# sashakolpakov/graphem-rapids

Hardware: AMD Instinct MI355X
Metric: layout iterations/s (higher is better)
Workload: dtype f32; 1 GPU; rr1m; graph=rr, n_vertices=1000000, n_edges=4000000, n_components=3, n_neighbors=10, sample_size=256, sampler=device, knn=auto, knn_distance=exact, parallelism=rows/1, reference_identical=False

## Files before the change

graphem-rapids_amd/csrc/common.h:

```cpp
#pragma once
#include <hip/hip_runtime.h>
#include <stdint.h>

#include "dispatch.h"

#define GH_WAVE 64
#ifndef GH_DEPTH8
#define GH_DEPTH8 4
#endif
#ifndef GH_DEPTH16
#define GH_DEPTH16 2
#endif
#define GH_GATHER_DEPTH(LD) ((LD) <= 4 ? 8 : (LD) <= 8 ? GH_DEPTH8 : GH_DEPTH16)

template <int D>
__device__ __forceinline__ float gh_sumsq(const float *x) {
    float s = 0.0f;
    int d = 0;
    if constexpr (D >= 8) {
        float acc[8];
#pragma unroll
        for (int l = 0; l < 8; ++l) acc[l] = 0.0f;
#pragma unroll
        for (d = 0; d + 8 <= D; d += 8) {
// ... 32 lines not shown
__device__ __forceinline__ void gh_load_row(const float *__restrict__ pos, int64_t v, float *out) {
    const float4 *p = reinterpret_cast<const float4 *>(pos + v * LD);
#pragma unroll
    for (int i = 0; i < LD / 4; ++i) {
        const float4 t = p[i];
        out[4 * i + 0] = t.x; out[4 * i + 1] = t.y; out[4 * i + 2] = t.z; out[4 * i + 3] = t.w;
    }
}

template <int LD>
__device__ __forceinline__ void gh_store_row(float *__restrict__ dst, int64_t v, const float *in) {
    float4 *p = reinterpret_cast<float4 *>(dst + v * LD);
#pragma unroll
    for (int i = 0; i < LD / 4; ++i) p[i] = make_float4(in[4 * i], in[4 * i + 1], in[4 * i + 2], in[4 * i + 3]);
}

__device__ __forceinline__ uint64_t gh_key(float d2, uint32_t id) {
    return (static_cast<uint64_t>(__float_as_uint(d2)) << 32) | id;
}
__device__ __forceinline__ float gh_key_d2(uint64_t k) { return __uint_as_float(static_cast<uint32_t>(k >> 32)); }
__device__ __forceinline__ uint32_t gh_key_id(uint64_t k) { return static_cast<uint32_t>(k); }

#define GH_KEY_INF 0xFFFFFFFFFFFFFFFFull

__device__ __forceinline__ double gh_wave_sum(double v) {
#pragma unroll
    for (int off = 32; off > 0; off >>= 1) v += __shfl_down(v, off, GH_WAVE);
    return v;
}

__device__ __forceinline__ float gh_sqrt_ieee(float x) {
    if (__builtin_expect(!(x >= 0x1p-96f), 0)) return sqrtf(x);
    const float s = __builtin_amdgcn_sqrtf(x);
    const float sm = __uint_as_float(__float_as_uint(s) - 1u), sp = __uint_as_float(__float_as_uint(s) + 1u);
    const float rm = fmaf(-sm, s, x), rp = fmaf(-sp, s, x);
    float out = rm <= 0.0f ? sm : s;
    out = rp > 0.0f ? sp : out;
    return x == INFINITY ? x : out;
}
template <int D>
__device__ __forceinline__ void gh_div_by(const float (&n)[D], float d, float (&q)[D]) {
    uint32_t emin = 255;
#pragma unroll
    for (int i = 0; i < D; ++i) emin = min(emin, (__float_as_uint(n[i]) >> 23) & 0xFFu);
    if (__builtin_expect(!(d >= 0x1p-40f && d <= 0x1p20f) || emin < 27u, 0)) {
#pragma unroll
// ... 144 lines not shown
```

graphem-rapids_amd/csrc/engine.h:

```cpp
#pragma once
#include <hip/hip_runtime.h>
#include <stdint.h>
#include <memory>
#include <string>
#include <vector>

#include "../../include/graphem_hip.h"
#include "host_util.h"
#include "step_plan.h"
#include "exchange_layout.h"

#define GH_CAND_CAP 16384
#define GH_SEL_BUF 4096
#define GH_SEL_CHUNK 2048
#define GH_CNT_STRIDE 32
#define GH_POS_PAD_ROWS 1024
#define GH_CT_M 64
#define GH_CT_EMPTY 0xFFFFFFFFu

struct gh_timer_slot {
    std::string name;
    double total_ms = 0.0;
    int64_t launches = 0;
    std::vector<std::pair<hipEvent_t, hipEvent_t>> pending;
// ... 145 lines not shown

    int grid_G = 0, grid_bits = 0;
    int64_t grid_cells = 0;
    size_t grid_temp_bytes = 0;
    gh_dev<uint32_t> d_grid_u32;
    gh_dev<float> d_grid_smid;
    gh_dev<unsigned char> d_grid_temp;

    gh_dev<double> d_blockstats;
    int nblocks_update = 0;
    gh_dev<double> d_stats_buf;
    double *d_stats = nullptr;

    gh_dev<unsigned> d_tau_flag;
    gh_dev<uint32_t> d_qcell;
    gh_dev<unsigned> d_qc_flag;
    unsigned qc_epoch = 0;
    gh_dev<int32_t> d_wait_failed;
    gh_dev<uint32_t> d_cmin;
    bool cmin_dirty[2] = {false, false};


#define GH_STAMP_EXTRA 8192
    gh_dev<unsigned long long> d_stamps;
    bool timing = false;
    std::vector<gh_timer_slot> timers;

    std::unique_ptr<gh_ivf, gh_part_delete> ivf;
    std::unique_ptr<gh_f64, gh_part_delete> f64;
    std::unique_ptr<gh_comm, gh_part_delete> comm;
};

template <class T> gh_status gh_alloc(gh_engine *h, gh_dev<T> &buf, size_t count, bool zero) {
    if (count == 0) count = 1;
    if (!buf.alloc(count * sizeof(T))) {
        h->err = std::string("hipMalloc failed: ") + hipGetErrorString(hipGetLastError());
        return GH_ERR_NOMEM;
    }
    if (zero) GH_HIP(hipMemsetAsync(buf.p, 0, count * sizeof(T), h->stream));
    return GH_OK;
}

inline gh_ids gh_own_ids(const gh_engine *h) { return gh_ids{h->S >= h->E ? GH_IDS_ARANGE : GH_IDS_SAMPLER, h->d_sampled.p}; }
inline void gh_set_lookahead(gh_engine *h, const gh_ids *next) {
    h->lookahead.valid = next != nullptr;
    h->lookahead.rows = false;
// ... 5 lines not shown
    h->lookahead.src = next;
    h->lookahead.iter = h->iter + 1;
}
inline bool gh_lookahead_rows_for(const gh_engine *h, const gh_ids *next) {
    return next && h->lookahead.rows && h->lookahead.iter == h->iter + 1 && h->lookahead.src.mode == next->mode &&
           h->lookahead.src.ids == next->ids;
}
inline void gh_drop_lookahead_rows(gh_engine *h) { h->lookahead.rows = false; }
inline bool gh_lookahead_done_for(const gh_engine *h, const gh_ids &src) {
    return h->lookahead.valid && h->lookahead.iter == h->iter && h->lookahead.src.mode == src.mode && h->lookahead.src.ids == src.ids;
}
inline void gh_drop_lookahead(gh_engine *h) { h->lookahead.valid = false; }

inline void gh_step_reset(gh_engine *h) {
    h->step.new0_ready = h->step.stats_reduced = h->step.intersect_done = h->step.rows_early = false;
}
inline void gh_step_new0_ready(gh_engine *h) { h->step.new0_ready = true; }
inline void gh_step_stats_reduced(gh_engine *h) { h->step.stats_reduced = true; }
inline void gh_step_sums_spent(gh_engine *h) { h->step.new0_ready = h->step.stats_reduced = false; }
inline void gh_step_intersect_done(gh_engine *h) { h->step.intersect_done = true; }
inline void gh_step_tcount_reset_pending(gh_engine *h, bool pending) { h->step.tcount_reset_pending = pending; }
inline void gh_step_set_rows_early(gh_engine *h, bool early) { h->step.rows_early = early; }
inline void gh_step_own_ids(gh_engine *h, bool own) { h->step.own_ids = own; }

enum gh_finish_kind { GH_FINISH_OWN, GH_FINISH_OWN_ALL_STATS, GH_FINISH_ALL_ROWS };

struct gh_scope {
    gh_engine *h;
    int slot = -1;
    hipEvent_t a = nullptr, b = nullptr;
    hipStream_t stream = nullptr;
    gh_scope(gh_engine *h_, const char *name, hipStream_t on = nullptr );
    ~gh_scope();
};

struct gh_graph_plan {
    const int32_t *edges = nullptr;
    std::vector<int32_t> internal;
    std::vector<int32_t> rowptr, adj;
    std::vector<int32_t> first_edge, own_eids, vblock;
    std::vector<int32_t> long_rows, long_ownptr, long_ownadj, long_eptr, long_erow;
    std::vector<uint8_t> own_long;
    std::vector<int32_t> sub_uv;
};
void gh_plan_graph(gh_engine *h, const int32_t *edges, bool partitioned, int reorder, gh_graph_plan *g);
void gh_auto_knn_method(gh_engine *h);
// ... 64 lines not shown
```

graphem-rapids_amd/csrc/forces.hip:

```cpp
#include "common.h"
#include "engine.h"
#include "intersect_core.h"
#include "setup_core.h"

namespace {

template <int D, int LD, bool WRITE_MID, bool LONG>
__global__ __launch_bounds__(256) void spring_kernel(
    const float *__restrict__ pos, const int32_t *__restrict__ rowptr, const int32_t *__restrict__ adj,
    const int32_t *__restrict__ first_edge, int64_t edge_lo, int64_t row_lo, int64_t rows, float L_min,
    float neg_k, float *__restrict__ outF, int64_t f_row0, float *__restrict__ mid, gh_long_args la) {
    const int64_t i = blockIdx.x * (int64_t)blockDim.x + threadIdx.x;
    if (i >= rows) return;
    const int64_t x = row_lo + i;
    float px[LD], F[LD];
    gh_load_row<LD>(pos, x, px);
    int64_t mid_row0 = 0;
    if (WRITE_MID) mid_row0 = first_edge[i] - edge_lo;
    if constexpr (LONG)
        spring_row<D, LD, WRITE_MID>(pos, adj, rowptr[i], rowptr[i + 1], x, px, L_min, neg_k, F, mid, mid_row0, la, (int)i,
                                     outF + (i + f_row0) * LD);
    else
        spring_pull<D, LD, WRITE_MID>(pos, adj, rowptr[i], rowptr[i + 1], x, px, L_min, neg_k, F, mid, mid_row0);
    gh_store_row<LD>(outF, i + f_row0, F);
// ... 196 lines not shown
__global__ __launch_bounds__(256) void stats_reduce_kernel(const double *__restrict__ blockstats, int nblocks, int LD,
                                                          double *__restrict__ stats) {
    const int c = blockIdx.x;
    double s = 0.0;
    for (int b = threadIdx.x; b < nblocks; b += blockDim.x) s += blockstats[(int64_t)c * nblocks + b];
    __shared__ double red[4];
    const double a = gh_wave_sum(s);
    if ((threadIdx.x & 63) == 0) red[threadIdx.x >> 6] = a;
    __syncthreads();
    if (threadIdx.x == 0) stats[c] = ((red[0] + red[1]) + red[2]) + red[3];
}

template <int LD>
__global__ __launch_bounds__(256) void stats_fix_kernel(const double *__restrict__ blockstats, int nblocks,
                                                       const float *__restrict__ pos, const float *__restrict__ Fs,
                                                       const double *__restrict__ acc,
                                                       const int32_t *__restrict__ touched,
                                                       const int32_t *__restrict__ tcount, int64_t row_lo,
                                                       int64_t rows, float *__restrict__ out_new,
                                                       double *__restrict__ stats, int skip_reduce,
                                                       int32_t *__restrict__ patch_count = nullptr ,
                                                       float *__restrict__ patch_rows = nullptr, int patch_cap = 0,
                                                       gh_setup_args sa = gh_setup_args{} ,
                                                       const int32_t *__restrict__ tflag = nullptr, float *__restrict__ setup_rows = nullptr) {
    constexpr int NFIX = 2 * LD;
    if ((int)blockIdx.x >= NFIX) {
        gh_setup_gather<LD>(sa, gh_gather_src{pos, Fs, out_new, acc, tflag, setup_rows}, (int)blockIdx.x - NFIX);
        return;
    }
    __shared__ double red[4][2 * LD];
    const int lane = threadIdx.x & 63, w = threadIdx.x >> 6;
    if (!skip_reduce) {
        const int c = blockIdx.x;
        double s = 0.0;
        double s4[4] = {0.0, 0.0, 0.0, 0.0};
        const double *col = blockstats + (int64_t)c * nblocks;
        int b = threadIdx.x;
        for (; b + 3 * (int)blockDim.x < nblocks; b += 4 * blockDim.x) {
#pragma unroll
            for (int u = 0; u < 4; ++u) s4[u] += col[b + u * blockDim.x];
        }
        for (int u = 0; b < nblocks; b += blockDim.x, ++u) s4[u] += col[b];
        s = (s4[0] + s4[1]) + (s4[2] + s4[3]);
        const double a = gh_wave_sum(s);
        if (lane == 0) red[w][0] = a;
        __syncthreads();
        if (threadIdx.x == 0) stats[c] = ((red[0][0] + red[1][0]) + red[2][0]) + red[3][0];
        __syncthreads();
    }
    double dx[LD], dxx[LD];
#pragma unroll
    for (int d = 0; d < LD; ++d) { dx[d] = 0.0; dxx[d] = 0.0; }
    const int nt = *tcount;
    for (int t = blockIdx.x * blockDim.x + threadIdx.x; t < nt; t += NFIX * blockDim.x) {
        const int64_t x = touched[t];
        const int64_t i = x - row_lo;
        if (i < 0 || i >= rows) continue;
        float p[LD], f[LD], nw[LD];
        gh_load_row<LD>(pos, x, p);
        gh_load_row<LD>(Fs, i, f);
#pragma unroll
        for (int d = 0; d < LD; ++d) {
            const float n0 = p[d] + f[d];
            const float tot = f[d] + (float)acc[x * LD + d];
            nw[d] = p[d] + tot;
            dx[d] += (double)nw[d] - (double)n0;
            dxx[d] += (double)nw[d] * (double)nw[d] - (double)n0 * (double)n0;
        }
        if (!patch_count) gh_store_row<LD>(out_new, i, nw);
        else gh_patch_append<LD>(patch_count, patch_rows, patch_cap, x, nw);
    }
#pragma unroll
    for (int d = 0; d < LD; ++d) {
        const double a = gh_wave_sum(dx[d]), b = gh_wave_sum(dxx[d]);
        if (lane == 0) { red[w][d] = a; red[w][LD + d] = b; }
    }
    __syncthreads();
    if (threadIdx.x < 2 * LD)
        stats[(2 + 2 * blockIdx.x) * LD + threadIdx.x] =
            ((red[0][threadIdx.x] + red[1][threadIdx.x]) + red[2][threadIdx.x]) + red[3][threadIdx.x];
}

__device__ __forceinline__ void gh_clear_touched(double *__restrict__ acc, int32_t *__restrict__ tflag,
                                                 const int32_t *__restrict__ touched, const int32_t *__restrict__ tcount, int LD,
                                                 int64_t t0, int64_t T) {
    const int64_t nt = (int64_t)(*tcount) * LD;
    for (int64_t t = t0; t < nt; t += T) {
        const int64_t x = touched[t / LD];
        const int d = (int)(t % LD);
        acc[x * LD + d] = 0.0;
        if (d == 0) tflag[x] = 0;
    }
}

struct gh_norm_src {
    const float *rows;
    int64_t chunk;
    int64_t block;
    int RS;
    int64_t out_lo, out_rows;
    const double *stats;
    int world;
    int64_t stats_block;
// ... 393 lines not shown
    }
    if (!fused) return launch_mid_gather(h);
    return GH_OK;
}

gh_status gh_launch_mid_only(gh_engine *h) { return launch_mid_gather(h); }

gh_status gh_launch_integrate(gh_engine *h, const gh_ids *next) {
    gh_drop_lookahead_rows(h);
    const bool fused_sums = h->step.new0_ready && h->rows > 0, reduced = h->step.stats_reduced;
    gh_step_sums_spent(h);
    if (fused_sums) {
        gh_scope t(h, "stats_fix");
        gh_setup_args sa{};
        unsigned gather = 0;
        if (next && h->plan.stage_rows) {
            sa = gh_make_setup_args(h, *next, h->iter + 1);
            if (sa.tiles > 0) gather = gh_gather_blocks(sa.S);
        }
        if (!gh_dispatch_stride(h->LD, [&](auto ld) {
                stats_fix_kernel<ld()><<<dim3(gh_fix_blocks(ld()) + gather), dim3(256), 0, h->stream>>>(
                    h->d_blockstats.p, h->n_vblocks, h->d_pos.p, h->d_Fs.p, h->d_acc.p, h->d_touched.p, h->d_tcount.p, h->part.row_lo,
                    h->rows, h->d_new, h->d_stats, reduced ? 1 : 0,
                    gh_patch_count(h), gh_patch_records(h), (int)h->xch.lay.patch_cap, sa, h->d_tflag.p, h->d_setup_rows.p);
            })) {
            h->err = "stats_fix: the fused step left its sums for a row stride other than 4, 8 or 16";
            return GH_ERR_RUNTIME;
        }
        GH_LAUNCH_CHECK();
        if (gather) gh_set_lookahead_rows(h, *next);
        return GH_OK;
    }
    GH_HIP(hipMemsetAsync(h->d_stats + 2 * h->LD, 0, sizeof(double) * 2 * gh_fix_blocks(h->LD) * h->LD, h->stream));
    if (h->rows == 0) {
        GH_HIP(hipMemsetAsync(h->d_stats, 0, sizeof(double) * 2 * h->LD, h->stream));
        return GH_OK;
    }
    const unsigned grid = grid_for(h->rows, 256);
    int32_t *pc = gh_patch_count(h);
    float *pr = gh_patch_records(h);
    const int pcap = (int)h->xch.lay.patch_cap;
    float *wide_out = h->d_new;
    {
        gh_scope t(h, "integrate");
        if (!gh_dispatch_stride(h->LD, [&](auto ld) {
                integrate_kernel<ld()><<<dim3(grid), dim3(256), 0, h->stream>>>(h->d_pos.p, h->d_Fs.p, h->part.row_lo, h->rows, h->d_acc.p,
                                                                               h->d_tflag.p, h->d_new, h->d_blockstats.p, pc, pr, pcap);
// ... 238 lines not shown
```

graphem-rapids_amd/csrc/intersect_core.h:

```cpp
#pragma once
#include "common.h"

__host__ __device__ __forceinline__ float gh_orient2d(const float *a, const float *b, const float *c) {
    return (b[0] - a[0]) * (c[1] - a[1]) - (b[1] - a[1]) * (c[0] - a[0]);
}

__device__ inline void gh_intersect_pair(const float *__restrict__ pos, int D, int LD,
                                         const int32_t *__restrict__ edges, int32_t i, int32_t j, float k_inter,
                                         double *__restrict__ acc, int32_t *__restrict__ tflag,
                                         int32_t *__restrict__ touched, int32_t *__restrict__ tcount,
                                         float *__restrict__ diff, int32_t own_lo = 0, int32_t own_hi = 0x7FFFFFFF ) {
    if (!(i < j)) return;
    const int32_t v[4] = {edges[2 * (int64_t)i], edges[2 * (int64_t)i + 1], edges[2 * (int64_t)j], edges[2 * (int64_t)j + 1]};
    if (v[0] == v[2] || v[0] == v[3] || v[1] == v[2] || v[1] == v[3]) return;
    if (D < 2) return;
    const float *p1 = pos + (int64_t)v[0] * LD, *p2 = pos + (int64_t)v[1] * LD;
    const float *q1 = pos + (int64_t)v[2] * LD, *q2 = pos + (int64_t)v[3] * LD;
    const float o1 = gh_orient2d(p1, p2, q1), o2 = gh_orient2d(p1, p2, q2);
    const float o3 = gh_orient2d(q1, q2, p1), o4 = gh_orient2d(q1, q2, p2);
    if (!(o1 * o2 < 0.0f && o3 * o4 < 0.0f)) return;
    for (int role = 0; role < 4; ++role) {
        if (v[role] < own_lo || v[role] >= own_hi) continue;
        const float *x = pos + (int64_t)v[role] * LD;
        for (int d = 0; d < D; ++d) {
// ... 33 lines not shown
        for (int d = 0; d < D; ++d) diff[d] = x[role][d] - cen[d];
        const float dist = sqrtf(gh_sumsq<D>(diff)) + 1e-6f;
        const float dd = dist * dist;
#pragma unroll
        for (int d = 0; d < D; ++d) atomicAdd(&acc[(int64_t)v[role] * LD + d], (double)((k_inter * diff[d]) / dd));
        if (atomicExch(&tflag[v[role]], 1) == 0) touched[atomicAdd(tcount, 1)] = v[role];
    }
}

struct gh_pair_list {
    int n;
    int nt, base;
    int4 v[128];
    int32_t t[512];
};

template <int D, int LD>
__device__ __forceinline__ void gh_intersect_query_wide(const float *__restrict__ pos, const int32_t *__restrict__ edges,
                                                        int32_t i, const uint64_t *best , int k,
                                                        float k_inter, double *__restrict__ acc,
                                                        int32_t *__restrict__ tflag, int32_t *__restrict__ touched,
                                                        int32_t *__restrict__ tcount, gh_pair_list *pl,
                                                        int32_t *__restrict__ own_count = nullptr ,
                                                        int32_t own_lo = 0, int32_t own_hi = 0x7FFFFFFF) {
    if (threadIdx.x == 0) { pl->n = 0; pl->nt = 0; }
    __syncthreads();
    for (int c = threadIdx.x; c < k; c += blockDim.x) {
        const int32_t j = (int32_t)(uint32_t)best[c + 1];
        if (!(i < j)) continue;
        const int2 ei = reinterpret_cast<const int2 *>(edges)[i], ej = reinterpret_cast<const int2 *>(edges)[j];
        if (ei.x == ej.x || ei.x == ej.y || ei.y == ej.x || ei.y == ej.y) continue;
        const float2 a = *reinterpret_cast<const float2 *>(pos + (int64_t)ei.x * LD), b = *reinterpret_cast<const float2 *>(pos + (int64_t)ei.y * LD);
        const float2 p = *reinterpret_cast<const float2 *>(pos + (int64_t)ej.x * LD), q = *reinterpret_cast<const float2 *>(pos + (int64_t)ej.y * LD);
        const float x0[2] = {a.x, a.y}, x1[2] = {b.x, b.y}, x2[2] = {p.x, p.y}, x3[2] = {q.x, q.y};
        const float o1 = gh_orient2d(x0, x1, x2), o2 = gh_orient2d(x0, x1, x3);
        const float o3 = gh_orient2d(x2, x3, x0), o4 = gh_orient2d(x2, x3, x1);
        if (!(o1 * o2 < 0.0f && o3 * o4 < 0.0f)) continue;
        pl->v[atomicAdd(&pl->n, 1)] = make_int4(ei.x, ei.y, ej.x, ej.y);
    }
    __syncthreads();
    constexpr int LPP = 4 * LD;
    const int np = pl->n;
    const int sub = threadIdx.x % LPP, role = sub / LD, d = sub % LD;
    for (int p = threadIdx.x / LPP; p < np; p += blockDim.x / LPP) {
        const int4 vv = pl->v[p];
        const int32_t v[4] = {vv.x, vv.y, vv.z, vv.w};
        float x[4][LD];
#pragma unroll
        for (int r = 0; r < 4; ++r) gh_load_row<LD>(pos, v[r], x[r]);
        float diff[D];
#pragma unroll
        for (int dd = 0; dd < D; ++dd) {
            const float cen = (((x[0][dd] + x[1][dd]) + x[2][dd]) + x[3][dd]) / 4.0f;
            const float mine = role == 0 ? x[0][dd] : role == 1 ? x[1][dd] : role == 2 ? x[2][dd] : x[3][dd];
            diff[dd] = mine - cen;
        }
        const float dist = sqrtf(gh_sumsq<D>(diff)) + 1e-6f;
        const float dsq = dist * dist;
        float term = diff[0];
#pragma unroll
        for (int dd = 1; dd < D; ++dd) term = d == dd ? diff[dd] : term;
        const int32_t me = role == 0 ? v[0] : role == 1 ? v[1] : role == 2 ? v[2] : v[3];
        if (me < own_lo || me >= own_hi) continue;
        if (d < D) atomicAdd(&acc[(int64_t)me * LD + d], (double)((k_inter * term) / dsq));
        if (d == 0 && atomicExch(&tflag[me], 1) == 0) pl->t[atomicAdd(&pl->nt, 1)] = me;
    }
    __syncthreads();
    const int nt = pl->nt;
    if (own_count) {
        if (threadIdx.x == 0) *own_count = nt;
        for (int i = threadIdx.x; i < nt; i += blockDim.x) touched[i] = pl->t[i];
        return;
    }
    if (nt == 0) return;
    if (threadIdx.x == 0) pl->base = atomicAdd(tcount, nt);
    __syncthreads();
    for (int i = threadIdx.x; i < nt; i += blockDim.x) touched[pl->base + i] = pl->t[i];
}

__device__ __forceinline__ void gh_intersect_pair_any(const float *__restrict__ pos, int D, int LD,
                                                      const int32_t *__restrict__ edges, int32_t i, int32_t j,
                                                      float k_inter, double *__restrict__ acc,
                                                      int32_t *__restrict__ tflag, int32_t *__restrict__ touched,
                                                      int32_t *__restrict__ tcount, float *__restrict__ diff) {
#define GH_INTERSECT_ONE(DD) \
    case DD: gh_intersect_pair_t<DD, gh_ld(DD)>(pos, edges, i, j, k_inter, acc, tflag, touched, tcount); break;
    switch (D) {
        GH_INTERSECT_ONE(2) GH_INTERSECT_ONE(3) GH_INTERSECT_ONE(4) GH_INTERSECT_ONE(5) GH_INTERSECT_ONE(6)
        GH_INTERSECT_ONE(7) GH_INTERSECT_ONE(8) GH_INTERSECT_ONE(9) GH_INTERSECT_ONE(10) GH_INTERSECT_ONE(11)
        GH_INTERSECT_ONE(12) GH_INTERSECT_ONE(13) GH_INTERSECT_ONE(14) GH_INTERSECT_ONE(15) GH_INTERSECT_ONE(16)
        default: gh_intersect_pair(pos, D, LD, edges, i, j, k_inter, acc, tflag, touched, tcount, diff);
    }
#undef GH_INTERSECT_ONE
}
```

graphem-rapids_amd/csrc/knn.hip:

```cpp
#include "common.h"
#include "engine.h"
#include "scan_core.h"
#include "setup_core.h"
#include "tau_core.h"
#include "intersect_core.h"
#include "select_core.h"

#include <math.h>
#include <type_traits>
#include <stdlib.h>

namespace {


template <bool COARSE>
__global__ __launch_bounds__(256) void knn_setup_kernel(const float *__restrict__ pos, gh_setup_args a,
                                                       int32_t *__restrict__ tcount, int32_t *__restrict__ qexact) {
    __shared__ __align__(16) unsigned char lds[GH_SETUP_LDS_BYTES];
    if (blockIdx.x == 0 && threadIdx.x == 0) { *tcount = 0; qexact[0] = 0; }
    const int LD = a.LD;
    auto getp = [=](int64_t v, int d) { return pos[v * LD + d]; };
    if constexpr (COARSE) gh_setup_block<4, true>(a, (int)blockIdx.x, getp, lds);
    else if (a.tiles > 0) gh_setup_block_any(a, (int)blockIdx.x, getp, lds);
    else gh_setup_item(a, blockIdx.x * (int64_t)blockDim.x + threadIdx.x, getp);
// ... 182 lines not shown
        if (r & 1) c0[r / 2].y = c; else c0[r / 2].x = c;
#pragma unroll
        for (int d = 0; d < D; ++d) {
            if (r & 1) m[r / 2][d].y = mv[d];
            else m[r / 2][d].x = mv[d];
        }
    }
    __syncthreads();
    gh_scan_queries<D, R, GH_SCAN_HITBUF>(m, c0, id, qsh, nq, s_lo, taush, hkey, hq, &hcount, cand, cnt, nullptr, cdist);
    __syncthreads();
    gh_flush_hits<GH_SCAN_HITBUF>(hkey, hq, &hcount, cand, cnt);
}

template <int NV, int FORM>
__global__ __launch_bounds__(64) void knn_tau_kernel(gh_tau_args a) { gh_tau_query_any<FORM, NV>(a, blockIdx.x, threadIdx.x); }

template <int DT>
__global__ __launch_bounds__(256) void knn_select_kernel(uint64_t *__restrict__ cand, int32_t *__restrict__ cnt,
                                                         int K, int final_level, float *__restrict__ tau, int QS,
                                                         uint64_t *__restrict__ out_keys,
                                                         int32_t *__restrict__ ovf, int32_t *__restrict__ dbg_cnt,
                                                         search_args fb, inter_args ia, int S,
                                                         const double *__restrict__ blockstats, int nblocks,
                                                         double *__restrict__ stats, int32_t *__restrict__ only = nullptr) {
    extern __shared__ __align__(16) unsigned char smem_raw[];
    float *qs = reinterpret_cast<float *>(smem_raw);
    __shared__ uint64_t best[GH_EXTRACT_MAX_K];
    __shared__ uint64_t best2[GH_EXTRACT_MAX_K];
    __shared__ uint64_t red[4 * GH_EXTRACT_MAX_K];
    static_assert(GH_CAND_CAP <= 2 * GH_LIST_HALF, "block_extract_list takes two halves");
    const int64_t qi = blockIdx.x;
    if (qi >= S) {
        gh_reduce_stats_column(blockstats, nblocks, (int)(qi - S), stats, reinterpret_cast<double *>(red));
        return;
    }
    if (only && !only[qi]) return;
    uint64_t pre[4];
#pragma unroll
    for (int j = 0; j < 4; ++j) pre[j] = cand[qi * GH_CAND_CAP + j * 256 + threadIdx.x];
    const int c = cnt[qi * GH_CNT_STRIDE];
    __syncthreads();
    if (threadIdx.x == 0) { cnt[qi * GH_CNT_STRIDE] = 0; dbg_cnt[qi] = c; if (only) only[qi] = 0; }
    if (__builtin_expect(c > GH_CAND_CAP || c < K, 0)) {
        if (!final_level) return;
        if (threadIdx.x == 0) ovf[qi] = 1;
        block_search_query(fb, qi, K, qs, best, red);
    } else if (c <= 1024 && !(K > 16 && c <= 512)) {
#pragma unroll
        for (int j = 0; j < 4; ++j) pre[j] = j * 256 + (int)threadIdx.x < c ? pre[j] : GH_KEY_INF;
        block_extract_smallest<4>(pre, K, best, red);
    } else {
        block_extract_list(cand + qi * GH_CAND_CAP, c, K, best, best2, red);
    }
    if (final_level) {
        for (int i = threadIdx.x; i < K; i += blockDim.x) out_keys[qi * K + i] = best[i];
        __shared__ gh_pair_list pairs;
        if (ia.pos) intersect_query<DT>(ia, qi, best, &pairs);
    } else if (threadIdx.x == 0) {
        tau[qi * QS] = gh_key_d2(best[K - 1]);
    }
}

template <int DT>
__global__ __launch_bounds__(64) void knn_select_wave_kernel(const uint64_t *__restrict__ cand, int32_t *__restrict__ cnt, int K,
                                                            uint64_t *__restrict__ out_keys, int32_t *__restrict__ dbg_cnt,
                                                            int32_t *__restrict__ redo, inter_args ia, int S) {
    constexpr int NT = 64;
    __shared__ uint64_t best[GH_EXTRACT_MAX_K];
    __shared__ uint64_t red[2 * NT];
    __shared__ gh_pair_list pairs;
    const int64_t qi = blockIdx.x;
    if (qi >= S) return;
    uint64_t pre[4];
#pragma unroll
    for (int j = 0; j < 4; ++j) pre[j] = cand[qi * GH_CAND_CAP + j * NT + threadIdx.x];
    const int c = cnt[qi * GH_CNT_STRIDE];
    if (c > 16 * NT || c < K) {
        if (threadIdx.x == 0) redo[qi] = 1;
        return;
    }
// ... 132 lines not shown
    }
}

gh_status launch_select(gh_engine *h, bool final_level, bool with_intersect, const float *fb_mid) {
    const bool reduce = final_level && gh_sums_ride_along(h->plan, h->step);
    gh_scope t(h, with_intersect ? "knn_select_intersect" : "knn_select");
    const bool wave = final_level && !reduce && h->S >= 2048;
    bool wave_tq = false;
    if (wave) {
        inter_args iaw = make_inter_args(h, with_intersect);
        wave_tq = with_intersect && h->k <= 127 && h->D >= 2 && h->LD <= 16;
        if (wave_tq) { iaw.tq_count = h->d_tq_count.p; iaw.tq_touched = h->d_tq_touched.p; }
        const auto select_wave = [&](auto d) {
            knn_select_wave_kernel<d()><<<dim3((unsigned)h->S), dim3(64), 0, h->stream>>>(
                h->d_cand.p, h->d_cnt.p, h->K, h->d_partial.p, h->d_dbg_cnt.p + (size_t)h->S, h->d_sel_redo.p, iaw, (int)h->S);
        };
        if (!(with_intersect && gh_dispatch_dim(h->D, [&](auto d, auto) { select_wave(d); }))) select_wave(gh_int<0>{});
    }
    const auto select = [&](auto d) {
        knn_select_kernel<d()><<<dim3((unsigned)h->S + (reduce ? 2u * (unsigned)h->LD : 0u)), dim3(256), sizeof(float) * (size_t)h->LD, h->stream>>>(
            h->d_cand.p, h->d_cnt.p, h->K, final_level ? 1 : 0, h->d_q.p + gh_qtau(h->D, h->LD), gh_qs(h->D, h->LD),
            h->d_partial.p, h->d_ovf.p, h->d_dbg_cnt.p + (size_t)(final_level ? 1 : 0) * h->S,
            make_search_args(h, fb_mid, h->own_count, 1, 1), make_inter_args(h, with_intersect), (int)h->S,
            h->d_blockstats.p, h->n_vblocks, h->d_stats, wave ? h->d_sel_redo.p : nullptr);
    };
    if (!(with_intersect && gh_dispatch_dim(h->D, [&](auto d, auto) { select(d); }))) select(gh_int<0>{});
    if (wave_tq) {
        const int k4 = 4 * h->k;
        knn_touched_prefix_kernel<<<dim3(1), dim3(1024), 0, h->stream>>>(h->d_tq_count.p, (int)h->S, h->d_tq_base.p, h->d_tcount.p);
        knn_touched_copy_kernel<<<dim3((unsigned)(((int64_t)h->S * k4 + 255) / 256)), dim3(256), 0, h->stream>>>(
            h->d_tq_count.p, h->d_tq_base.p, h->d_tq_touched.p, (int)h->S, k4, h->d_touched.p);
        GH_HIP(hipMemsetAsync(h->d_tq_count.p, 0, sizeof(int32_t) * (size_t)h->S, h->stream));
    }
    GH_LAUNCH_CHECK();
    if (reduce) gh_step_stats_reduced(h);
    return GH_OK;
}

}

gh_setup_args gh_make_setup_args(const gh_engine *h, gh_ids src, uint64_t iter) {
    const int tiles = (int)((h->plan.thr_M1 + GH_THR_TILE - 1) / GH_THR_TILE);
    return gh_setup_args{h->d_edges.p, src.ids, src.mode, h->E, h->prm.seed, iter, h->S, h->D, h->LD, h->d_q.p, h->d_cnt.p,
                         h->d_ovf.p, h->part.edge_lo, h->d_own_eids.p, reinterpret_cast<const int2 *>(h->d_sub_uv.p), h->plan.thr_M1, h->plan.thr_stride, h->d_gmin.p,
                         (int64_t)tiles * GH_THR_GROUPS, tiles, h->plan.tau == GH_TAUF_EMBEDDED ? h->d_tau_flag.p : nullptr,
                         nullptr ,
                         h->plan.tau == GH_TAUF_COARSE && tiles > 0 ? h->d_cmin.p + (size_t)(iter & 1) * GH_CT_M * (size_t)h->S : nullptr};
// ... 202 lines not shown
```

graphem-rapids_amd/csrc/select_core.h:

```cpp
#pragma once
#include "common.h"
#include "engine.h"
#include "intersect_core.h"
#include <type_traits>

namespace {

struct inter_args {
    const float *pos;
    const int32_t *edges;
    const int32_t *sampled;
    int D, LD, k;
    float k_inter;
    double *acc;
    int32_t *tflag, *touched, *tcount;
    float *scratch;
    int32_t *tq_count = nullptr;
    int32_t *tq_touched = nullptr;
    int32_t own_lo = 0, own_hi = 0x7FFFFFFF;
};

template <int DT>
__device__ __forceinline__ void intersect_query(const inter_args &ia, int64_t qi, const uint64_t *best, gh_pair_list *pl) {
    if constexpr (DT >= 2) {
        constexpr int LL = gh_ld(DT);
        if (ia.k <= 127 && blockDim.x % (4 * LL) == 0) {
            if (ia.tq_count)
                gh_intersect_query_wide<DT, LL>(ia.pos, ia.edges, ia.sampled[qi], best, ia.k, ia.k_inter, ia.acc, ia.tflag,
                                                ia.tq_touched + qi * 4 * ia.k, ia.tcount, pl, ia.tq_count + qi, ia.own_lo, ia.own_hi);
            else
                gh_intersect_query_wide<DT, LL>(ia.pos, ia.edges, ia.sampled[qi], best, ia.k, ia.k_inter, ia.acc, ia.tflag, ia.touched,
                                                ia.tcount, pl, nullptr, ia.own_lo, ia.own_hi);
            return;
        }
    }
    for (int c = threadIdx.x; c < ia.k; c += blockDim.x) {
        const int32_t j = (int32_t)gh_key_id(best[c + 1]);
        if constexpr (DT >= 2)
            gh_intersect_pair_t<DT, gh_ld(DT)>(ia.pos, ia.edges, ia.sampled[qi], j, ia.k_inter, ia.acc, ia.tflag,
                                               ia.touched, ia.tcount, ia.own_lo, ia.own_hi);
        else
            gh_intersect_pair(ia.pos, ia.D, ia.LD, ia.edges, ia.sampled[qi], j, ia.k_inter, ia.acc, ia.tflag, ia.touched, ia.tcount,
                              ia.scratch + (qi * ia.k + c) * ia.LD, ia.own_lo, ia.own_hi);
    }
}

__device__ __forceinline__ void block_sort(uint64_t *buf, int n2) {
    for (int k = 2; k <= n2; k <<= 1) {
        for (int j = k >> 1; j > 0; j >>= 1) {
            for (int i = threadIdx.x; i < n2; i += blockDim.x) {
                const int ixj = i ^ j;
                if (ixj > i) {
                    const uint64_t a = buf[i], b = buf[ixj];
                    const bool asc = (i & k) == 0;
                    if ((a > b) == asc) { buf[i] = b; buf[ixj] = a; }
                }
            }
            __syncthreads();
        }
    }
}

__device__ __forceinline__ int next_pow2(int x) {
    int p = 1;
    while (p < x) p <<= 1;
    return p;
}

template <int CTRL>
__device__ __forceinline__ uint64_t dpp_u64(uint64_t v) {
    int lo = (int)(uint32_t)v, hi = (int)(uint32_t)(v >> 32);
    lo = __builtin_amdgcn_update_dpp(lo, lo, CTRL, 0xF, 0xF, false);
    hi = __builtin_amdgcn_update_dpp(hi, hi, CTRL, 0xF, 0xF, false);
    return ((uint64_t)(uint32_t)hi << 32) | (uint32_t)lo;
}
__device__ __forceinline__ uint64_t readlane_u64(uint64_t v, int lane) {
    const uint32_t lo = (uint32_t)__builtin_amdgcn_readlane((int)(uint32_t)v, lane);
    const uint32_t hi = (uint32_t)__builtin_amdgcn_readlane((int)(uint32_t)(v >> 32), lane);
    return ((uint64_t)hi << 32) | lo;
}
__device__ __forceinline__ uint64_t min_u64(uint64_t a, uint64_t b) { return b < a ? b : a; }
__device__ __forceinline__ uint64_t wave_min_u64(uint64_t v) {
    v = min_u64(v, dpp_u64<0xB1>(v));
    v = min_u64(v, dpp_u64<0x4E>(v));
    v = min_u64(v, dpp_u64<0x141>(v));
    v = min_u64(v, dpp_u64<0x140>(v));
    return min_u64(min_u64(readlane_u64(v, 0), readlane_u64(v, 16)),
                   min_u64(readlane_u64(v, 32), readlane_u64(v, 48)));
}


template <int NPT, int NT = 256>
__device__ __forceinline__ void block_extract_smallest(uint64_t (&keys)[NPT], int K, uint64_t *out, uint64_t *wsc) {
    const int lane = threadIdx.x & 63, w = threadIdx.x >> 6;
    for (int r = 0; r < K; ++r) {
        uint64_t m = keys[0];
#pragma unroll
        for (int j = 1; j < NPT; ++j) m = min_u64(m, keys[j]);
        m = wave_min_u64(m);
        if (lane == 0) wsc[w * K + r] = m;
        if (m == GH_KEY_INF) {
            for (int rr = r + 1 + lane; rr < K; rr += 64) wsc[w * K + rr] = GH_KEY_INF;
            break;
        }
#pragma unroll
        for (int j = 0; j < NPT; ++j) keys[j] = keys[j] == m ? GH_KEY_INF : keys[j];
    }
    __syncthreads();
    const int n4 = (NT / 64) * K;
    for (int t = threadIdx.x; t < n4; t += NT) {
        const uint64_t key = wsc[t];
        int rank = 0;
        for (int j = 0; j < n4; ++j) {
            const uint64_t o = wsc[j];
            rank += (o < key || (o == key && j < t)) ? 1 : 0;
        }
        if (rank < K) out[rank] = key;
    }
    __syncthreads();
}



template <int NT = 256>
__device__ __forceinline__ void block_rank_smallest(const uint64_t *src, int c, int K, uint64_t *out, uint64_t *stage ) {
    uint64_t mine[2];
#pragma unroll
    for (int j = 0; j < 2; ++j) {
        const int i = j * NT + threadIdx.x;
        mine[j] = i < c ? src[i] : GH_KEY_INF;
        stage[i] = mine[j];
    }
    for (int i = c + threadIdx.x; i < K; i += NT) out[i] = GH_KEY_INF;
    __syncthreads();
    int rank[2] = {0, 0};
    const int c2 = (c + 1) & ~1;
    for (int i = 0; i < c2; i += 2) {
        const uint64_t a = stage[i], b = stage[i + 1];
#pragma unroll
        for (int j = 0; j < 2; ++j) rank[j] += (a < mine[j] ? 1 : 0) + (b < mine[j] ? 1 : 0);
    }
#pragma unroll
// ... 76 lines not shown
```

Before: 6702 iterations/s.

## Fuse top-K extraction merge with intersection pass and add per-workgroup timing stamps

Adds a merged path to the final-level selection kernel. Each wave's extracted top-K lists are ranked directly, and the edge-intersection check runs from those ranks without first materialising a sorted best[] array, with neighbour edge rows prefetched during extraction. It also rewrites the 64-bit wave min as two 32-bit DPP min passes in inline asm, and widens the candidate preload to 8 per thread to handle counts up to 2048 in registers. It also adds wall-clock stamp instrumentation to the selection and stats_fix kernels; these stamps only fire when a stamp buffer is allocated, but they add extra arguments and branches. The aim is to cut shared-memory round trips and syncs between selection and intersection, at the cost of more registers and more shared memory for pair rows.

```diff
diff --git a/graphem-rapids_amd/csrc/common.h b/graphem-rapids_amd/csrc/common.h
--- a/graphem-rapids_amd/csrc/common.h
+++ b/graphem-rapids_amd/csrc/common.h
@@ -78,6 +78,8 @@
 __device__ __forceinline__ uint32_t gh_key_id(uint64_t k) { return static_cast<uint32_t>(k); }
 
 #define GH_KEY_INF 0xFFFFFFFFFFFFFFFFull
+
+#define GH_WG_STAMP(st, k) do { if ((st) && threadIdx.x == 0) { asm volatile("s_waitcnt vmcnt(0)" ::: "memory"); (st)[k] = wall_clock64(); } } while (0)
 
 __device__ __forceinline__ double gh_wave_sum(double v) {
 #pragma unroll
diff --git a/graphem-rapids_amd/csrc/engine.h b/graphem-rapids_amd/csrc/engine.h
--- a/graphem-rapids_amd/csrc/engine.h
+++ b/graphem-rapids_amd/csrc/engine.h
@@ -191,6 +191,10 @@
 
 
 #define GH_STAMP_EXTRA 8192
+#define GH_SEL_STAMP_FIRST 4096
+#define GH_SEL_STAMP_MAX 1024
+#define GH_FIX_STAMP_FIRST 5120
+#define GH_FIX_STAMP_MAX 64
     gh_dev<unsigned long long> d_stamps;
     bool timing = false;
     std::vector<gh_timer_slot> timers;
@@ -242,6 +246,12 @@
 inline void gh_step_tcount_reset_pending(gh_engine *h, bool pending) { h->step.tcount_reset_pending = pending; }
 inline void gh_step_set_rows_early(gh_engine *h, bool early) { h->step.rows_early = early; }
 inline void gh_step_own_ids(gh_engine *h, bool own) { h->step.own_ids = own; }
+
+inline unsigned long long *gh_extra_stamps(gh_engine *h, int first) {
+    return h->d_stamps.p ? h->d_stamps.p + ((int64_t)std::max(h->n_vblocks, 1) + first) * 8 : nullptr;
+}
+inline unsigned long long *gh_select_stamps(gh_engine *h) { return gh_extra_stamps(h, GH_SEL_STAMP_FIRST); }
+inline unsigned long long *gh_fix_stamps(gh_engine *h) { return gh_extra_stamps(h, GH_FIX_STAMP_FIRST); }
 
 enum gh_finish_kind { GH_FINISH_OWN, GH_FINISH_OWN_ALL_STATS, GH_FINISH_ALL_ROWS };
 
diff --git a/graphem-rapids_amd/csrc/forces.hip b/graphem-rapids_amd/csrc/forces.hip
--- a/graphem-rapids_amd/csrc/forces.hip
+++ b/graphem-rapids_amd/csrc/forces.hip
@@ -242,10 +242,15 @@
                                                        int32_t *__restrict__ patch_count = nullptr ,
                                                        float *__restrict__ patch_rows = nullptr, int patch_cap = 0,
                                                        gh_setup_args sa = gh_setup_args{} ,
-                                                       const int32_t *__restrict__ tflag = nullptr, float *__restrict__ setup_rows = nullptr) {
+                                                       const int32_t *__restrict__ tflag = nullptr, float *__restrict__ setup_rows = nullptr,
+                                                       unsigned long long *__restrict__ stamps = nullptr ) {
     constexpr int NFIX = 2 * LD;
+    if (stamps) stamps = blockIdx.x < GH_FIX_STAMP_MAX ? stamps + (int64_t)blockIdx.x * 8 : nullptr;
+    GH_WG_STAMP(stamps, 0);
+    if (stamps && threadIdx.x == 0) { stamps[2] = stamps[3] = 0; stamps[7] = (int)blockIdx.x >= NFIX ? 5u : 4u; }
     if ((int)blockIdx.x >= NFIX) {
         gh_setup_gather<LD>(sa, gh_gather_src{pos, Fs, out_new, acc, tflag, setup_rows}, (int)blockIdx.x - NFIX);
+        GH_WG_STAMP(stamps, 4);
         return;
     }
     __shared__ double red[4][2 * LD];
@@ -272,8 +277,10 @@
 #pragma unroll
     for (int d = 0; d < LD; ++d) { dx[d] = 0.0; dxx[d] = 0.0; }
     const int nt = *tcount;
+    GH_WG_STAMP(stamps, 1);
     for (int t = blockIdx.x * blockDim.x + threadIdx.x; t < nt; t += NFIX * blockDim.x) {
         const int64_t x = touched[t];
+        GH_WG_STAMP(stamps, 2);
         const int64_t i = x - row_lo;
         if (i < 0 || i >= rows) continue;
         float p[LD], f[LD], nw[LD];
@@ -287,6 +294,7 @@
             dx[d] += (double)nw[d] - (double)n0;
             dxx[d] += (double)nw[d] * (double)nw[d] - (double)n0 * (double)n0;
         }
+        GH_WG_STAMP(stamps, 3);
         if (!patch_count) gh_store_row<LD>(out_new, i, nw);
         else gh_patch_append<LD>(patch_count, patch_rows, patch_cap, x, nw);
     }
@@ -299,6 +307,7 @@
     if (threadIdx.x < 2 * LD)
         stats[(2 + 2 * blockIdx.x) * LD + threadIdx.x] =
             ((red[0][threadIdx.x] + red[1][threadIdx.x]) + red[2][threadIdx.x]) + red[3][threadIdx.x];
+    GH_WG_STAMP(stamps, 4);
 }
 
 __device__ __forceinline__ void gh_clear_touched(double *__restrict__ acc, int32_t *__restrict__ tflag,
@@ -738,7 +747,8 @@
                 stats_fix_kernel<ld()><<<dim3(gh_fix_blocks(ld()) + gather), dim3(256), 0, h->stream>>>(
                     h->d_blockstats.p, h->n_vblocks, h->d_pos.p, h->d_Fs.p, h->d_acc.p, h->d_touched.p, h->d_tcount.p, h->part.row_lo,
                     h->rows, h->d_new, h->d_stats, reduced ? 1 : 0,
-                    gh_patch_count(h), gh_patch_records(h), (int)h->xch.lay.patch_cap, sa, h->d_tflag.p, h->d_setup_rows.p);
+                    gh_patch_count(h), gh_patch_records(h), (int)h->xch.lay.patch_cap, sa, h->d_tflag.p, h->d_setup_rows.p,
+                    gh_fix_stamps(h));
             })) {
             h->err = "stats_fix: the fused step left its sums for a row stride other than 4, 8 or 16";
             return GH_ERR_RUNTIME;
diff --git a/graphem-rapids_amd/csrc/intersect_core.h b/graphem-rapids_amd/csrc/intersect_core.h
--- a/graphem-rapids_amd/csrc/intersect_core.h
+++ b/graphem-rapids_amd/csrc/intersect_core.h
@@ -79,13 +79,15 @@
                                                         int32_t *__restrict__ tflag, int32_t *__restrict__ touched,
                                                         int32_t *__restrict__ tcount, gh_pair_list *pl,
                                                         int32_t *__restrict__ own_count = nullptr ,
-                                                        int32_t own_lo = 0, int32_t own_hi = 0x7FFFFFFF) {
+                                                        int32_t own_lo = 0, int32_t own_hi = 0x7FFFFFFF,
+                                                        unsigned long long *st = nullptr ) {
     if (threadIdx.x == 0) { pl->n = 0; pl->nt = 0; }
     __syncthreads();
     for (int c = threadIdx.x; c < k; c += blockDim.x) {
         const int32_t j = (int32_t)(uint32_t)best[c + 1];
         if (!(i < j)) continue;
         const int2 ei = reinterpret_cast<const int2 *>(edges)[i], ej = reinterpret_cast<const int2 *>(edges)[j];
+        GH_WG_STAMP(st, 3);
         if (ei.x == ej.x || ei.x == ej.y || ei.y == ej.x || ei.y == ej.y) continue;
         const float2 a = *reinterpret_cast<const float2 *>(pos + (int64_t)ei.x * LD), b = *reinterpret_cast<const float2 *>(pos + (int64_t)ei.y * LD);
         const float2 p = *reinterpret_cast<const float2 *>(pos + (int64_t)ej.x * LD), q = *reinterpret_cast<const float2 *>(pos + (int64_t)ej.y * LD);
@@ -96,6 +98,7 @@
         pl->v[atomicAdd(&pl->n, 1)] = make_int4(ei.x, ei.y, ej.x, ej.y);
     }
     __syncthreads();
+    GH_WG_STAMP(st, 4);
     constexpr int LPP = 4 * LD;
     const int np = pl->n;
     const int sub = threadIdx.x % LPP, role = sub / LD, d = sub % LD;
@@ -123,6 +126,7 @@
         if (d == 0 && atomicExch(&tflag[me], 1) == 0) pl->t[atomicAdd(&pl->nt, 1)] = me;
     }
     __syncthreads();
+    GH_WG_STAMP(st, 5);
     const int nt = pl->nt;
     if (own_count) {
         if (threadIdx.x == 0) *own_count = nt;
@@ -132,6 +136,7 @@
     if (nt == 0) return;
     if (threadIdx.x == 0) pl->base = atomicAdd(tcount, nt);
     __syncthreads();
+    GH_WG_STAMP(st, 6);
     for (int i = threadIdx.x; i < nt; i += blockDim.x) touched[pl->base + i] = pl->t[i];
 }
 
diff --git a/graphem-rapids_amd/csrc/knn.hip b/graphem-rapids_amd/csrc/knn.hip
--- a/graphem-rapids_amd/csrc/knn.hip
+++ b/graphem-rapids_amd/csrc/knn.hip
@@ -228,7 +228,8 @@
                                                          int32_t *__restrict__ ovf, int32_t *__restrict__ dbg_cnt,
                                                          search_args fb, inter_args ia, int S,
                                                          const double *__restrict__ blockstats, int nblocks,
-                                                         double *__restrict__ stats, int32_t *__restrict__ only = nullptr) {
+                                                         double *__restrict__ stats, int32_t *__restrict__ only = nullptr,
+                                                         unsigned long long *__restrict__ stamps = nullptr ) {
     extern __shared__ __align__(16) unsigned char smem_raw[];
     float *qs = reinterpret_cast<float *>(smem_raw);
     __shared__ uint64_t best[GH_EXTRACT_MAX_K];
@@ -241,27 +242,61 @@
         return;
     }
     if (only && !only[qi]) return;
-    uint64_t pre[4];
-#pragma unroll
-    for (int j = 0; j < 4; ++j) pre[j] = cand[qi * GH_CAND_CAP + j * 256 + threadIdx.x];
+    if (stamps) stamps = qi < GH_SEL_STAMP_MAX ? stamps + qi * 8 : nullptr;
+    GH_WG_STAMP(stamps, 0);
+    const bool merged = DT >= 2 && final_level && ia.pos && ia.k <= 127 && K <= 64;
+    const int32_t si = merged ? ia.sampled[qi] : 0;
+    uint64_t pre[8];
+#pragma unroll
+    for (int j = 0; j < 8; ++j) pre[j] = cand[qi * GH_CAND_CAP + j * 256 + threadIdx.x];
     const int c = cnt[qi * GH_CNT_STRIDE];
+    const int2 sei = merged ? reinterpret_cast<const int2 *>(ia.edges)[si] : make_int2(0, 0);
+    bool in_red = false;
+    int32_t warm = 0;
+    const int32_t *warm_src = merged ? ia.edges : cnt + qi * GH_CNT_STRIDE;
+    const auto own = [&](bool mine, uint64_t m) {
+        const int32_t j = (int32_t)(uint32_t)m;
+        warm = warm_src[merged ? 2 * (int64_t)(mine && si < j ? j : si) : 0];
+    };
     __syncthreads();
     if (threadIdx.x == 0) { cnt[qi * GH_CNT_STRIDE] = 0; dbg_cnt[qi] = c; if (only) only[qi] = 0; }
+    if (stamps && threadIdx.x == 0) stamps[7] = ((unsigned long long)(unsigned)c << 8) | 3u;
+    GH_WG_STAMP(stamps, 1);
     if (__builtin_expect(c > GH_CAND_CAP || c < K, 0)) {
         if (!final_level) return;
         if (threadIdx.x == 0) ovf[qi] = 1;
         block_search_query(fb, qi, K, qs, best, red);
-    } else if (c <= 1024 && !(K > 16 && c <= 512)) {
-#pragma unroll
-        for (int j = 0; j < 4; ++j) pre[j] = j * 256 + (int)threadIdx.x < c ? pre[j] : GH_KEY_INF;
-        block_extract_smallest<4>(pre, K, best, red);
+    } else if (K > 16 && c <= 512) {
+        block_extract_list(cand + qi * GH_CAND_CAP, c, K, best, best2, red);
+    } else if (c <= 1024) {
+        uint64_t (&pre4)[4] = reinterpret_cast<uint64_t (&)[4]>(pre);
+#pragma unroll
+        for (int j = 0; j < 4; ++j) pre4[j] = j * 256 + (int)threadIdx.x < c ? pre4[j] : GH_KEY_INF;
+        block_extract_rounds<4>(pre4, K, red, own);
+        in_red = true;
+    } else if (c <= 2048) {
+#pragma unroll
+        for (int j = 0; j < 8; ++j) pre[j] = j * 256 + (int)threadIdx.x < c ? pre[j] : GH_KEY_INF;
+        block_extract_rounds<8>(pre, K, red, own);
+        in_red = true;
     } else {
         block_extract_list(cand + qi * GH_CAND_CAP, c, K, best, best2, red);
     }
+    GH_WG_STAMP(stamps, 2);
+    __shared__ gh_pair_list pairs;
+    if (in_red) {
+        if constexpr (DT >= 2) {
+            if (merged) {
+                __shared__ gh_pair_rows<gh_ld(DT)> prows;
+                gh_merge_intersect_query<DT, gh_ld(DT)>(ia, qi, K, red, out_keys, si, sei, warm, &pairs, &prows, stamps);
+                return;
+            }
+        }
+        block_extract_merge(K, best, red);
+    }
     if (final_level) {
         for (int i = threadIdx.x; i < K; i += blockDim.x) out_keys[qi * K + i] = best[i];
-        __shared__ gh_pair_list pairs;
-        if (ia.pos) intersect_query<DT>(ia, qi, best, &pairs);
+        if (ia.pos) intersect_query<DT>(ia, qi, best, &pairs, stamps);
     } else if (threadIdx.x == 0) {
         tau[qi * QS] = gh_key_d2(best[K - 1]);
     }
@@ -440,7 +475,8 @@
             h->d_cand.p, h->d_cnt.p, h->K, final_level ? 1 : 0, h->d_q.p + gh_qtau(h->D, h->LD), gh_qs(h->D, h->LD),
             h->d_partial.p, h->d_ovf.p, h->d_dbg_cnt.p + (size_t)(final_level ? 1 : 0) * h->S,
             make_search_args(h, fb_mid, h->own_count, 1, 1), make_inter_args(h, with_intersect), (int)h->S,
-            h->d_blockstats.p, h->n_vblocks, h->d_stats, wave ? h->d_sel_redo.p : nullptr);
+            h->d_blockstats.p, h->n_vblocks, h->d_stats, wave ? h->d_sel_redo.p : nullptr,
+            final_level ? gh_select_stamps(h) : nullptr);
     };
     if (!(with_intersect && gh_dispatch_dim(h->D, [&](auto d, auto) { select(d); }))) select(gh_int<0>{});
     if (wave_tq) {
diff --git a/graphem-rapids_amd/csrc/select_core.h b/graphem-rapids_amd/csrc/select_core.h
--- a/graphem-rapids_amd/csrc/select_core.h
+++ b/graphem-rapids_amd/csrc/select_core.h
@@ -21,16 +21,17 @@
 };
 
 template <int DT>
-__device__ __forceinline__ void intersect_query(const inter_args &ia, int64_t qi, const uint64_t *best, gh_pair_list *pl) {
+__device__ __forceinline__ void intersect_query(const inter_args &ia, int64_t qi, const uint64_t *best, gh_pair_list *pl,
+                                                unsigned long long *st = nullptr ) {
     if constexpr (DT >= 2) {
         constexpr int LL = gh_ld(DT);
         if (ia.k <= 127 && blockDim.x % (4 * LL) == 0) {
             if (ia.tq_count)
                 gh_intersect_query_wide<DT, LL>(ia.pos, ia.edges, ia.sampled[qi], best, ia.k, ia.k_inter, ia.acc, ia.tflag,
-                                                ia.tq_touched + qi * 4 * ia.k, ia.tcount, pl, ia.tq_count + qi, ia.own_lo, ia.own_hi);
+                                                ia.tq_touched + qi * 4 * ia.k, ia.tcount, pl, ia.tq_count + qi, ia.own_lo, ia.own_hi, st);
             else
                 gh_intersect_query_wide<DT, LL>(ia.pos, ia.edges, ia.sampled[qi], best, ia.k, ia.k_inter, ia.acc, ia.tflag, ia.touched,
-                                                ia.tcount, pl, nullptr, ia.own_lo, ia.own_hi);
+                                                ia.tcount, pl, nullptr, ia.own_lo, ia.own_hi, st);
             return;
         }
     }
@@ -67,33 +68,45 @@
     return p;
 }
 
-template <int CTRL>
-__device__ __forceinline__ uint64_t dpp_u64(uint64_t v) {
-    int lo = (int)(uint32_t)v, hi = (int)(uint32_t)(v >> 32);
-    lo = __builtin_amdgcn_update_dpp(lo, lo, CTRL, 0xF, 0xF, false);
-    hi = __builtin_amdgcn_update_dpp(hi, hi, CTRL, 0xF, 0xF, false);
-    return ((uint64_t)(uint32_t)hi << 32) | (uint32_t)lo;
-}
 __device__ __forceinline__ uint64_t readlane_u64(uint64_t v, int lane) {
     const uint32_t lo = (uint32_t)__builtin_amdgcn_readlane((int)(uint32_t)v, lane);
     const uint32_t hi = (uint32_t)__builtin_amdgcn_readlane((int)(uint32_t)(v >> 32), lane);
     return ((uint64_t)hi << 32) | lo;
 }
 __device__ __forceinline__ uint64_t min_u64(uint64_t a, uint64_t b) { return b < a ? b : a; }
+__device__ __forceinline__ uint32_t wave_min_u32(uint32_t v) {
+    uint32_t r = v;
+    asm("s_nop 1\n\t"
+        "v_min_u32_dpp %0, %0, %0 quad_perm:[1,0,3,2] row_mask:0xf bank_mask:0xf\n\t"
+        "s_nop 1\n\t"
+        "v_min_u32_dpp %0, %0, %0 quad_perm:[2,3,0,1] row_mask:0xf bank_mask:0xf\n\t"
+        "s_nop 1\n\t"
+        "v_min_u32_dpp %0, %0, %0 row_half_mirror row_mask:0xf bank_mask:0xf\n\t"
+        "s_nop 1\n\t"
+        "v_min_u32_dpp %0, %0, %0 row_mirror row_mask:0xf bank_mask:0xf\n\t"
+        "s_nop 0"
+        : "+v"(r));
+    const uint32_t a = (uint32_t)__builtin_amdgcn_readlane((int)r, 0), b = (uint32_t)__builtin_amdgcn_readlane((int)r, 16);
+    const uint32_t c = (uint32_t)__builtin_amdgcn_readlane((int)r, 32), d = (uint32_t)__builtin_amdgcn_readlane((int)r, 48);
+    const uint32_t ab = a < b ? a : b, cd = c < d ? c : d;
+    return ab < cd ? ab : cd;
+}
 __device__ __forceinline__ uint64_t wave_min_u64(uint64_t v) {
-    v = min_u64(v, dpp_u64<0xB1>(v));
-    v = min_u64(v, dpp_u64<0x4E>(v));
-    v = min_u64(v, dpp_u64<0x141>(v));
-    v = min_u64(v, dpp_u64<0x140>(v));
-    return min_u64(min_u64(readlane_u64(v, 0), readlane_u64(v, 16)),
-                   min_u64(readlane_u64(v, 32), readlane_u64(v, 48)));
-}
-
-
-template <int NPT, int NT = 256>
-__device__ __forceinline__ void block_extract_smallest(uint64_t (&keys)[NPT], int K, uint64_t *out, uint64_t *wsc) {
+    const uint32_t hi = (uint32_t)(v >> 32), lo = (uint32_t)v;
+    const uint32_t mh = wave_min_u32(hi);
+    const uint32_t ml = wave_min_u32(hi == mh ? lo : 0xFFFFFFFFu);
+    return ((uint64_t)mh << 32) | ml;
+}
+
+
+struct gh_no_owner { __device__ __forceinline__ void operator()(bool, uint64_t) const {} };
+template <int NPT, class Own = gh_no_owner>
+__device__ __forceinline__ void block_extract_rounds(uint64_t (&keys)[NPT], int K, uint64_t *wsc, Own own = Own{}) {
     const int lane = threadIdx.x & 63, w = threadIdx.x >> 6;
+    bool mine = false;
+    uint64_t prev = GH_KEY_INF;
     for (int r = 0; r < K; ++r) {
+        if constexpr (!std::is_same<Own, gh_no_owner>::value) own(mine, prev);
         uint64_t m = keys[0];
 #pragma unroll
         for (int j = 1; j < NPT; ++j) m = min_u64(m, keys[j]);
@@ -103,21 +116,125 @@
             for (int rr = r + 1 + lane; rr < K; rr += 64) wsc[w * K + rr] = GH_KEY_INF;
             break;
         }
-#pragma unroll
-        for (int j = 0; j < NPT; ++j) keys[j] = keys[j] == m ? GH_KEY_INF : keys[j];
-    }
+        mine = false;
+#pragma unroll
+        for (int j = 0; j < NPT; ++j) {
+            const bool hit = keys[j] == m;
+            mine |= hit;
+            keys[j] = hit ? GH_KEY_INF : keys[j];
+        }
+        prev = m;
+    }
+}
+__device__ __forceinline__ int block_extract_rank(const uint64_t *wsc, int n4, int t, uint64_t key) {
+    int rank = 0;
+    for (int j = 0; j < n4; ++j) {
+        const uint64_t o = wsc[j];
+        rank += (o < key || (o == key && j < t)) ? 1 : 0;
+    }
+    return rank;
+}
+template <int NT = 256>
+__device__ __forceinline__ void block_extract_merge(int K, uint64_t *out, const uint64_t *wsc) {
     __syncthreads();
     const int n4 = (NT / 64) * K;
     for (int t = threadIdx.x; t < n4; t += NT) {
         const uint64_t key = wsc[t];
-        int rank = 0;
-        for (int j = 0; j < n4; ++j) {
-            const uint64_t o = wsc[j];
-            rank += (o < key || (o == key && j < t)) ? 1 : 0;
-        }
+        const int rank = block_extract_rank(wsc, n4, t, key);
         if (rank < K) out[rank] = key;
     }
     __syncthreads();
+}
+template <int NPT, int NT = 256>
+__device__ __forceinline__ void block_extract_smallest(uint64_t (&keys)[NPT], int K, uint64_t *out, uint64_t *wsc) {
+    block_extract_rounds<NPT>(keys, K, wsc);
+    block_extract_merge<NT>(K, out, wsc);
+}
+
+template <int LD>
+struct gh_pair_rows { float x[128][2][LD]; };
+
+template <int D, int LD>
+__device__ __forceinline__ void gh_merge_intersect_query(const inter_args &ia, int64_t qi, int K, const uint64_t *wsc,
+                                                         uint64_t *__restrict__ out_keys, int32_t i, int2 ei,
+                                                         int32_t warm ,
+                                                         gh_pair_list *pl, gh_pair_rows<LD> *pr, unsigned long long *st) {
+    const int lane = threadIdx.x & 63, w = threadIdx.x >> 6, slot = w * K + lane;
+    const int2 *edges2 = reinterpret_cast<const int2 *>(ia.edges);
+    asm volatile("s_waitcnt lgkmcnt(0)" ::: "memory");
+    uint64_t key = GH_KEY_INF;
+    int2 ej = make_int2(0, 0);
+    if (lane < K) {
+        key = wsc[slot];
+        if (key != GH_KEY_INF && i < (int32_t)(uint32_t)key) ej = edges2[(uint32_t)key];
+    }
+    float xa[LD], xb[LD];
+    gh_load_row<LD>(ia.pos, ei.x, xa);
+    gh_load_row<LD>(ia.pos, ei.y, xb);
+    if (threadIdx.x == 0) { pl->n = 0; pl->nt = 0; }
+    __syncthreads();
+    int rank = K;
+    if (lane < K) {
+        rank = block_extract_rank(wsc, 4 * K, slot, key);
+        if (rank < K) out_keys[qi * K + rank] = key;
+    }
+    GH_WG_STAMP(st, 3);
+    asm volatile("" : : "v"(warm));
+    if (rank >= 1 && rank < K && rank <= ia.k && key != GH_KEY_INF) {
+        const int32_t j = (int32_t)(uint32_t)key;
+        if (i < j && !(ei.x == ej.x || ei.x == ej.y || ei.y == ej.x || ei.y == ej.y)) {
+            float xp[LD], xq[LD];
+            gh_load_row<LD>(ia.pos, ej.x, xp);
+            gh_load_row<LD>(ia.pos, ej.y, xq);
+            const float o1 = gh_orient2d(xa, xb, xp), o2 = gh_orient2d(xa, xb, xq);
+            const float o3 = gh_orient2d(xp, xq, xa), o4 = gh_orient2d(xp, xq, xb);
+            if (o1 * o2 < 0.0f && o3 * o4 < 0.0f) {
+                const int s = atomicAdd(&pl->n, 1);
+                pl->v[s] = make_int4(ei.x, ei.y, ej.x, ej.y);
+#pragma unroll
+                for (int d = 0; d < LD; ++d) { pr->x[s][0][d] = xp[d]; pr->x[s][1][d] = xq[d]; }
+            }
+        }
+    }
+    __syncthreads();
+    GH_WG_STAMP(st, 4);
+    constexpr int LPP = 4 * LD;
+    const int np = pl->n;
+    const int sub = threadIdx.x % LPP, role = sub / LD, d = sub % LD;
+    for (int p = threadIdx.x / LPP; p < np; p += blockDim.x / LPP) {
+        const int4 vv = pl->v[p];
+        const int32_t v[4] = {vv.x, vv.y, vv.z, vv.w};
+        const float *xp = pr->x[p][0], *xq = pr->x[p][1];
+        float diff[D];
+#pragma unroll
+        for (int dd = 0; dd < D; ++dd) {
+            const float cen = (((xa[dd] + xb[dd]) + xp[dd]) + xq[dd]) / 4.0f;
+            const float mine = role == 0 ? xa[dd] : role == 1 ? xb[dd] : role == 2 ? xp[dd] : xq[dd];
+            diff[dd] = mine - cen;
+        }
+        const float dist = sqrtf(gh_sumsq<D>(diff)) + 1e-6f;
+        const float dsq = dist * dist;
+        float term = diff[0];
+#pragma unroll
+        for (int dd = 1; dd < D; ++dd) term = d == dd ? diff[dd] : term;
+        const int32_t me = role == 0 ? v[0] : role == 1 ? v[1] : role == 2 ? v[2] : v[3];
+        if (me < ia.own_lo || me >= ia.own_hi) continue;
+        if (d < D) atomicAdd(&ia.acc[(int64_t)me * LD + d], (double)((ia.k_inter * term) / dsq));
+        if (d == 0 && atomicExch(&ia.tflag[me], 1) == 0) pl->t[atomicAdd(&pl->nt, 1)] = me;
+    }
+    __syncthreads();
+    GH_WG_STAMP(st, 5);
+    const int nt = pl->nt;
+    if (ia.tq_count) {
+        if (threadIdx.x == 0) ia.tq_count[qi] = nt;
+        for (int t = threadIdx.x; t < nt; t += blockDim.x) ia.tq_touched[qi * 4 * ia.k + t] = pl->t[t];
+        return;
+    }
+    if (nt == 0) return;
+    if (threadIdx.x == 0) pl->base = atomicAdd(ia.tcount, nt);
+    __syncthreads();
+    GH_WG_STAMP(st, 6);
+    for (int t = threadIdx.x; t < nt; t += blockDim.x) ia.touched[pl->base + t] = pl->t[t];
 }
 
 
```

Result: no change. 6749 iterations/s, median of 5 (+0.7%).
